# WestlyPark/StyleRenderer

Measured on AMD Instinct MI355X. Metric: generator fwd+bwd images/sec at 256^2, higher is better.
Workload: dtype f32

## Files before the change

stylerenderer_amd/csrc/conv_wino.hip:

```cpp
#include <type_traits>
#include "mfma_tile.h"
#include "conv_wino.h"
#include <cstdlib>

namespace {

__device__ __attribute__((aligned(16))) const float g_wino_zero[4] = {0.f, 0.f, 0.f, 0.f};

constexpr int TW = 16, TH = 4;
constexpr int NB = 64;
constexpr int EH = 2 * TH + 2;
constexpr int LEAD = 3;
constexpr int EWP = 40;
constexpr int PLANE = EH * EWP;

#ifdef WINO_TIMING
__device__ long long g_wino_stamps[8 * 16384];
#define WINO_STAMP(i) do { if (tid == 0) { g_wino_stamps[(blockIdx.x & 16383) * 8 + (i)] = wall_clock64(); } } while (0)
#else
#define WINO_STAMP(i)
#endif

template <int KC>
struct WG {
    static constexpr int CQ = KC / 4;
    static constexpr int PPS = CQ * 512;
    static constexpr int UV = 8 * PPS;
    static constexpr int U_INSTR = UV / 256;
    static constexpr int D_FLOATS = KC * PLANE;
    static constexpr int D_INSTR = (D_FLOATS / 4 + 63) / 64;
    static constexpr int D_BUF = D_INSTR * 256;
    static constexpr int D_PER_WAVE = (D_INSTR + 3) / 4;
    static constexpr int PAD = 4 * UV + 2 * D_BUF;
    static constexpr int STY = PAD + 3 * 256;
};

template <int KC>
__global__ __launch_bounds__(256) void k_conv_wino(const WinoParams p) {
#if __HIP_DEVICE_COMPILE__
    using G = WG<KC>;
    extern __shared__ __attribute__((aligned(16))) float smem[];
    float* const ubuf = smem;
    float* const vbuf = smem + 2 * G::UV;
    float* const dbuf = smem + 4 * G::UV + 1;
    float* const sty = smem + G::STY;

    int bid = sr_xcd_chunk(blockIdx.x, gridDim.x);
    const int slice = bid % p.ks;
    bid /= p.ks;
    const int n_t = bid % p.tiles_n;
    bid /= p.tiles_n;
    const int tx_i = bid % p.tiles_x;
    bid /= p.tiles_x;
    const int ty_i = bid % p.tiles_y;
    const int b = bid / p.tiles_y;
    const int oy0 = ty_i * (2 * TH), ox0 = tx_i * (2 * TW), n0 = n_t * NB;

    const int tid = threadIdx.x, lane = tid & 63;
    const int wave = __builtin_amdgcn_readfirstlane(tid >> 6);
    const int half = lane >> 5, l31 = lane & 31;
    const int wn = wave & 1, wt = wave >> 1;
    const int nchunks = p.kchunks;
    const int k_lo = slice * p.kchunks;
    const int all_chunks = p.C / KC;
    WINO_STAMP(0);
#ifdef WINO_TIMING
    const long long wino_c0 = clock64();
    if (tid == 0) {
        g_wino_stamps[(blockIdx.x & 16383) * 8 + 6] = __builtin_amdgcn_s_getreg((31 << 11) | 4);
        g_wino_stamps[(blockIdx.x & 16383) * 8 + 7] = __builtin_amdgcn_s_getreg((31 << 11) | 20);
    }
#endif

    int d_off[G::D_PER_WAVE];
#pragma unroll
    for (int i = 0; i < G::D_PER_WAVE; ++i) {
        const int j = wave + 4 * i;
        const int f = (j * 64 + lane) * 4;
        int off = SR_BUF_OOB;
        if (j < G::D_INSTR && f < G::D_FLOATS) {
            const int c = f / PLANE, q = f % PLANE;
            const int r = q / EWP, cola = q % EWP;
            const int gy = oy0 - 1 + r, gx = ox0 - 4 + cola;
            if (gy >= 0 && gy < p.H && gx >= 0 && gx + 3 < p.W) off = ((c * p.H + gy) * p.W + gx) * 4;
        }
        d_off[i] = off;
    }
    const int chunk_in_bytes = KC * p.H * p.W * 4;
    const __amdgpu_buffer_rsrc_t r_in = __builtin_amdgcn_make_buffer_rsrc(
        const_cast<float*>(p.in + ((int64_t)b * p.C + (int64_t)k_lo * KC) * p.H * p.W), 0, nchunks * chunk_in_bytes,
        SR_BUF_RSRC_WORD3);
    const __amdgpu_buffer_rsrc_t r_u = __builtin_amdgcn_make_buffer_rsrc(
        const_cast<float*>(p.u + ((int64_t)n_t * all_chunks + k_lo) * G::UV), 0, nchunks * G::UV * 4, SR_BUF_RSRC_WORD3);
    const int u_voff = lane * 16;

    auto dma_d1 = [&](int k, int buf, int i) {
        const int j = wave + 4 * i;
        float* dst = j < G::D_INSTR ? dbuf + buf * G::D_BUF + j * 256 : smem + G::PAD + (wave - 1) * 256;
        __builtin_amdgcn_raw_ptr_buffer_load_lds(r_in, (lptr_t)dst, 16, d_off[i], k * chunk_in_bytes, 0, 0);
    };
    auto dma_u1 = [&](int k, int buf, int i) {
        const int j = wave + 4 * i;
        __builtin_amdgcn_raw_ptr_buffer_load_lds(r_u, (lptr_t)(ubuf + buf * G::UV + j * 256), 16, u_voff,
                                                 (k * G::UV + j * 256) * 4, 0, 0);
    };
    auto dma_d = [&](int k, int buf) {
#pragma unroll
        for (int i = 0; i < G::D_PER_WAVE; ++i) dma_d1(k, buf, i);
    };
    auto dma_u = [&](int k, int buf) {
#pragma unroll
        for (int i = 0; i < G::U_INSTR / 4; ++i) dma_u1(k, buf, i);
    };

    static_assert(KC == 8, "two channel quads per chunk");
    const int t_cq = wave & 1, t_h = wave >> 1;
    const int t_ca = 4 * t_cq + t_h;
    const int t_rd = t_ca * PLANE + (2 * (lane >> 4)) * EWP + LEAD + 2 * (lane & 15);
    const int t_wr = t_cq * 512 + t_h * 128 + lane * 2;

    typedef float f2 __attribute__((ext_vector_type(2)));
    auto ld2 = [](const float* q) { return *reinterpret_cast<const f2*>(q); };
    auto st2 = [](float* q, f2 v) { *reinterpret_cast<f2*>(q) = v; };
    auto pk_add = [](f2 x, f2 y) { f2 r; asm("v_pk_add_f32 %0, %1, %2" : "=v"(r) : "v"(x), "v"(y)); return r; };
    auto pk_sub = [](f2 x, f2 y) {
        f2 r;
        asm("v_pk_add_f32 %0, %1, %2 neg_lo:[0,1] neg_hi:[0,1]" : "=v"(r) : "v"(x), "v"(y));
        return r;
    };
    auto pk_mul_s = [](f2 x, f2 sv, int ch) {
        f2 r;
        if (ch == 0) asm("v_pk_mul_f32 %0, %1, %2 op_sel:[0,0] op_sel_hi:[1,0]" : "=v"(r) : "v"(x), "v"(sv));
        else asm("v_pk_mul_f32 %0, %1, %2 op_sel:[0,1] op_sel_hi:[1,1]" : "=v"(r) : "v"(x), "v"(sv));
        return r;
    };
    auto pk_fms_s = [](f2 x, f2 sv, f2 y, int ch) {
        f2 r;
        if (ch == 0)
            asm("v_pk_fma_f32 %0, %1, %2, %3 op_sel:[0,0,0] op_sel_hi:[1,0,1] neg_lo:[0,0,1] neg_hi:[0,0,1]"
                : "=v"(r) : "v"(x), "v"(sv), "v"(y));
        else
            asm("v_pk_fma_f32 %0, %1, %2, %3 op_sel:[0,1,0] op_sel_hi:[1,1,1] neg_lo:[0,0,1] neg_hi:[0,0,1]"
                : "=v"(r) : "v"(x), "v"(sv), "v"(y));
        return r;
    };
    auto pk_fnma_s = [](f2 x, f2 sv, f2 y, int ch) {
        f2 r;
        if (ch == 0)
            asm("v_pk_fma_f32 %0, %1, %2, %3 op_sel:[0,0,0] op_sel_hi:[1,0,1] neg_lo:[1,0,0] neg_hi:[1,0,0]"
                : "=v"(r) : "v"(x), "v"(sv), "v"(y));
        else
            asm("v_pk_fma_f32 %0, %1, %2, %3 op_sel:[0,1,0] op_sel_hi:[1,1,1] neg_lo:[1,0,0] neg_hi:[1,0,0]"
                : "=v"(r) : "v"(x), "v"(sv), "v"(y));
        return r;
    };
    auto col01 = [](f2 tp, f2 tq) {
        f2 r;
        asm("v_pk_add_f32 %0, %1, %2 op_sel:[0,0] op_sel_hi:[1,0] neg_lo:[0,1] neg_hi:[0,0]" : "=v"(r) : "v"(tp), "v"(tq));
        return r;
    };
    auto col23 = [](f2 tp, f2 tq) {
        f2 r;
        asm("v_pk_add_f32 %0, %1, %2 op_sel:[0,1] op_sel_hi:[1,1] neg_lo:[0,1] neg_hi:[1,0]" : "=v"(r) : "v"(tq), "v"(tp));
        return r;
    };
    struct XF {
        f2 P[2][4], Q[2][4];
        f2 sp[2][2], sq[2][2];
        f2 tp[2][4], tq[2][4];
        f2 o01[2][4], o23[2][4];
    };
    auto xf_read = [&](XF& x, const float* d0, int r) {
#pragma unroll
        for (int ch = 0; ch < 2; ++ch) {
            x.P[ch][r] = ld2(d0 + ch * 2 * PLANE + r * EWP);
            x.Q[ch][r] = ld2(d0 + ch * 2 * PLANE + r * EWP + 2);
        }
    };
    auto xf_step = [&](XF& x, int step, f2 sv) {
#pragma unroll
        for (int ch = 0; ch < 2; ++ch) {
            if (step == 0) {
                x.sp[ch][0] = pk_mul_s(x.P[ch][1], sv, ch);
                x.sp[ch][1] = pk_mul_s(x.P[ch][2], sv, ch);
                x.sq[ch][0] = pk_mul_s(x.Q[ch][1], sv, ch);
                x.sq[ch][1] = pk_mul_s(x.Q[ch][2], sv, ch);
                x.tp[ch][0] = pk_fms_s(x.P[ch][0], sv, x.sp[ch][1], ch);
                x.tq[ch][0] = pk_fms_s(x.Q[ch][0], sv, x.sq[ch][1], ch);
            } else if (step == 1) {
                x.tp[ch][1] = pk_add(x.sp[ch][0], x.sp[ch][1]);
                x.tq[ch][1] = pk_add(x.sq[ch][0], x.sq[ch][1]);
                x.tp[ch][2] = pk_sub(x.sp[ch][1], x.sp[ch][0]);
                x.tq[ch][2] = pk_sub(x.sq[ch][1], x.sq[ch][0]);
                x.tp[ch][3] = pk_fnma_s(x.P[ch][3], sv, x.sp[ch][0], ch);
                x.tq[ch][3] = pk_fnma_s(x.Q[ch][3], sv, x.sq[ch][0], ch);
            } else {
#pragma unroll
                for (int q = 2 * (step - 2); q < 2 * (step - 2) + 2; ++q) {
                    x.o01[ch][q] = col01(x.tp[ch][q], x.tq[ch][q]);
                    x.o23[ch][q] = col23(x.tp[ch][q], x.tq[ch][q]);
                }
            }
        }
    };
    auto xf_write = [&](const XF& x, float* vout, int q) {
#pragma unroll
        for (int ch = 0; ch < 2; ++ch) {
            st2(vout + (2 * q) * G::PPS + ch * 256, x.o01[ch][q]);
            st2(vout + (2 * q + 1) * G::PPS + ch * 256, x.o23[ch][q]);
        }
    };
    auto transform = [&](int k, int dsel, int vsel) {
        const float* d0 = dbuf + dsel * G::D_BUF + t_rd;
        float* v = vbuf + vsel * G::UV + t_wr;
        f2 sv;
        sv.x = sty[k * KC + t_ca];
        sv.y = sty[k * KC + t_ca + 2];
        XF x;
#pragma unroll
        for (int r = 0; r < 4; ++r) xf_read(x, d0, r);
#pragma unroll
        for (int st = 0; st < 4; ++st) xf_step(x, st, sv);
#pragma unroll
        for (int q = 0; q < 4; ++q) xf_write(x, v, q);
    };

    f32x16 acc[16];
#pragma unroll
    for (int pos = 0; pos < 16; ++pos)
#pragma unroll
        for (int r = 0; r < 16; ++r) acc[pos][r] = 0.0f;

    const int a_off = (half * 64 + wn * 32 + l31) * 2;
    const int b_off = (half * 64 + wt * 32 + l31) * 2;

    dma_d(0, 0);
    dma_u(0, 0);
    if (nchunks > 1) dma_d(1, 1);
    for (int c = tid; c < nchunks * KC; c += 256)
        sty[c] = p.iscale ? p.iscale[(int64_t)b * p.C + k_lo * KC + c] : 1.0f;
    __builtin_amdgcn_s_waitcnt(0x0F70);
    __syncthreads();
    WINO_STAMP(1);
    transform(0, 0, 0);
    WINO_STAMP(2);

    static_assert(KC == 8, "the slot schedule below is written for two channel quads per chunk");
    f2 au[2][2][8], bv[2][2][8];
    auto mfma_step = [&](int cq, int m) {
        const int e = m >> 4, pos = m & 15, pp = pos >> 1;
        if (pos & 1) acc[pos] = __builtin_amdgcn_mfma_f32_32x32x2f32(au[cq][e][pp].y, bv[cq][e][pp].y, acc[pos], 0, 0, 0);
        else acc[pos] = __builtin_amdgcn_mfma_f32_32x32x2f32(au[cq][e][pp].x, bv[cq][e][pp].x, acc[pos], 0, 0, 0);
    };
    auto body = [&](int k, auto first_tag) {
        constexpr bool FIRST = decltype(first_tag)::value;
        __builtin_amdgcn_s_waitcnt(0x0F70);
        __syncthreads();
        const int kd = min(k + 2, nchunks - 1), ku = min(k + 1, nchunks - 1);
        const float* ub = ubuf + (k & 1) * G::UV + a_off;
        const float* vb_ = vbuf + (k & 1) * G::UV + b_off;
        const int kn = (k + 1 < nchunks) ? k + 1 : k;
        const float* d0 = dbuf + ((k + 1) & 1) * G::D_BUF + t_rd;
        float* vout = vbuf + ((k + 1) & 1) * G::UV + t_wr;
        f2 sab;
        sab.x = sty[kn * KC + t_ca];
        sab.y = sty[kn * KC + t_ca + 2];
        XF x;
        auto load_ops = [&](int cq, int pp) {
#pragma unroll
            for (int e = 0; e < 2; ++e) {
                au[cq][e][pp] = ld2(ub + pp * G::PPS + cq * 512 + e * 256);
                bv[cq][e][pp] = ld2(vb_ + pp * G::PPS + cq * 512 + e * 256);
            }
        };
#ifndef WINO_RD
#define WINO_RD "0123"
#define WINO_ST "4567"
#define WINO_WR "CDEF"
#define WINO_L0 "4567"
#define WINO_L1 "89AB"
#define WINO_DD "45"
#define WINO_DU "89AB"
#endif
        constexpr char RD[] = WINO_RD, ST[] = WINO_ST, WR[] = WINO_WR, L0[] = WINO_L0, L1[] = WINO_L1, DD[] = WINO_DD,
                       DU[] = WINO_DU;
        static_assert(sizeof(RD) == 5 && sizeof(ST) == 5 && sizeof(WR) == 5 && sizeof(L0) == 5 && sizeof(L1) == 5 &&
                      sizeof(DD) == 3 && sizeof(DU) == 5, "schedule strings");
        static_assert(G::D_PER_WAVE == 4 && G::U_INSTR / 4 == 8, "4 halo + 8 weight DMA instructions per wave");
#pragma unroll
        for (int s = 0; s < 16; ++s) {
            const int cq = (s < 8) ? 1 : 0, j = s & 7;
            const char d = s < 10 ? '0' + s : 'A' + (s - 10);
            if (!(FIRST && s < 8)) {
#pragma unroll
                for (int u = 0; u < 4; ++u) mfma_step(cq, 4 * j + u);
            }
#pragma unroll
            for (int i = 0; i < 4; ++i) {
                if (L0[i] == d) { load_ops(0, 2 * i); load_ops(0, 2 * i + 1); }
                if (L1[i] == d) { load_ops(1, 2 * i); load_ops(1, 2 * i + 1); }
            }
#ifndef WINO_NO_DMA
#pragma unroll
            for (int i = 0; i < 4; ++i) {
                if (i < 2 && DD[i] == d) { dma_d1(kd, k & 1, 2 * i); dma_d1(kd, k & 1, 2 * i + 1); }
                if (DU[i] == d) { dma_u1(ku, (k + 1) & 1, 2 * i); dma_u1(ku, (k + 1) & 1, 2 * i + 1); }
            }
#endif
#ifndef WINO_NO_XFORM
#pragma unroll
            for (int i = 0; i < 4; ++i) if (RD[i] == d) xf_read(x, d0, i);
#pragma unroll
            for (int i = 0; i < 4; ++i) if (ST[i] == d) xf_step(x, i, sab);
#pragma unroll
            for (int i = 0; i < 4; ++i) if (WR[i] == d) xf_write(x, vout, i);
#endif
            __builtin_amdgcn_sched_barrier(0);
        }
    };
    body(0, std::true_type{});
    for (int k = 1; k < nchunks; ++k) body(k, std::false_type{});
#pragma unroll
    for (int m = 0; m < 32; ++m) mfma_step(1, m);

    __builtin_amdgcn_s_waitcnt(0x0F70);
    WINO_STAMP(3);

    const int tile = wt * 32 + l31;
    const int oy = oy0 + 2 * (tile >> 4), ox = ox0 + 2 * (tile & 15);
    const int64_t plane = (int64_t)p.H * p.W;
    float nzv[2][2] = {{0.0f, 0.0f}, {0.0f, 0.0f}};
    if (p.nba && p.nz) {
#pragma clang fp contract(off)
        const float nw = p.nz_w[0];
        const float* nzp = p.nz + b * p.nz_bstride + (int64_t)oy * p.W + ox;
#pragma unroll
        for (int a = 0; a < 2; ++a) {
            nzv[a][0] = nw * nzp[a * p.W];
            nzv[a][1] = nw * nzp[a * p.W + 1];
        }
    }
#pragma unroll
    for (int r = 0; r < 16; ++r) {
        const int n = sr_mfma32_row(r, half, n0 + wn * 32);
        float s[2][4];
#pragma unroll
        for (int j = 0; j < 4; ++j) {
            const float m0 = acc[j][r], m1 = acc[4 + j][r], m2 = acc[8 + j][r], m3 = acc[12 + j][r];
            s[0][j] = (m0 + m1) + m2;
            s[1][j] = (m1 - m2) - m3;
        }
        if (p.ks > 1) {
            float* o = p.partial + (((int64_t)slice * p.B + b) * p.N + n) * plane + (int64_t)oy * p.W + ox;
            *reinterpret_cast<float2*>(o) = make_float2((s[0][0] + s[0][1]) + s[0][2], (s[0][1] - s[0][2]) - s[0][3]);
            *reinterpret_cast<float2*>(o + p.W) = make_float2((s[1][0] + s[1][1]) + s[1][2], (s[1][1] - s[1][2]) - s[1][3]);
            continue;
        }
        const float os = p.oscale ? p.oscale[(int64_t)b * p.N + n] : 1.0f;
        const float ob = p.obias ? p.obias[n] : 0.0f;
        float* o = p.out + ((int64_t)b * p.N + n) * plane + (int64_t)oy * p.W + ox;
        const float ab = (p.nba && p.abias) ? p.abias[n] : 0.0f;
        float y[2][2];
#pragma unroll
        for (int a = 0; a < 2; ++a) {
            const float y0 = (s[a][0] + s[a][1]) + s[a][2];
            const float y1 = (s[a][1] - s[a][2]) - s[a][3];
            float v0 = y0 * os + ob, v1 = y1 * os + ob;
            if (p.nba) {
#pragma clang fp contract(off)
                v0 = v0 + nzv[a][0];
                v1 = v1 + nzv[a][1];
                v0 = v0 + ab;
                v1 = v1 + ab;
                v0 = ((v0 > 0.0f) ? v0 : v0 * p.alpha) * p.gain;
                v1 = ((v1 > 0.0f) ? v1 : v1 * p.alpha) * p.gain;
            }
            y[a][0] = v0;
            y[a][1] = v1;
        }
        *reinterpret_cast<float2*>(o) = make_float2(y[0][0], y[0][1]);
        *reinterpret_cast<float2*>(o + p.W) = make_float2(y[1][0], y[1][1]);
    }
    WINO_STAMP(4);
#ifdef WINO_TIMING
    if (tid == 0) g_wino_stamps[(blockIdx.x & 16383) * 8 + 5] = clock64() - wino_c0;
#endif
#endif
}

__global__ __launch_bounds__(256) void k_wino_reduce(const WinoParams p) {
    const int64_t plane = (int64_t)p.H * p.W, total4 = (int64_t)p.B * p.N * plane / 4;
    const int64_t slab4 = total4;
    for (int64_t i = (int64_t)blockIdx.x * 256 + threadIdx.x; i < total4; i += (int64_t)gridDim.x * 256) {
        const float4* src = reinterpret_cast<const float4*>(p.partial) + i;
        float4 a = src[0];
        for (int s = 1; s < p.ks; ++s) {
            const float4 q = src[s * slab4];
            a.x += q.x; a.y += q.y; a.z += q.z; a.w += q.w;
        }
        const int64_t row = (i * 4) / plane;
        const int n = (int)(row % p.N), b = (int)(row / p.N);
        const int64_t pix = i * 4 - row * plane;
        const float os = p.oscale ? p.oscale[row] : 1.0f;
        const float ob = p.obias ? p.obias[n] : 0.0f;
        float v[4] = {a.x * os + ob, a.y * os + ob, a.z * os + ob, a.w * os + ob};
        if (p.nba) {
#pragma clang fp contract(off)
            const float ab = p.abias ? p.abias[n] : 0.0f;
            float nz[4] = {0.0f, 0.0f, 0.0f, 0.0f};
            if (p.nz) {
                const float nw = p.nz_w[0];
                const float4 q = *reinterpret_cast<const float4*>(p.nz + b * p.nz_bstride + pix);
                nz[0] = nw * q.x; nz[1] = nw * q.y; nz[2] = nw * q.z; nz[3] = nw * q.w;
            }
#pragma unroll
            for (int j = 0; j < 4; ++j) {
                float t = v[j] + nz[j];
                t = t + ab;
                v[j] = ((t > 0.0f) ? t : t * p.alpha) * p.gain;
            }
        }
        reinterpret_cast<float4*>(p.out)[i] = make_float4(v[0], v[1], v[2], v[3]);
    }
}

template <int KC>
__global__ __launch_bounds__(64) void k_wino_weights(float* __restrict__ u, const float* __restrict__ wt, int C,
                                                     int N, int ldw) {
    using G = WG<KC>;
    const int n = blockIdx.x * 64 + threadIdx.x, c = blockIdx.y;
    float g[3][3];
#pragma unroll
    for (int t = 0; t < 9; ++t) g[t / 3][t % 3] = wt[((int64_t)t * C + c) * ldw + n];
    float h[4][3];
#pragma unroll
    for (int j = 0; j < 3; ++j) {
        h[0][j] = g[0][j];
        h[1][j] = 0.5f * ((g[0][j] + g[2][j]) + g[1][j]);
        h[2][j] = 0.5f * ((g[0][j] + g[2][j]) - g[1][j]);
        h[3][j] = g[2][j];
    }
    const int cl = c % KC, cq = cl / 4, e = (cl % 4) / 2, hh = cl % 2;
    float* dst = u + ((int64_t)blockIdx.x * (C / KC) + c / KC) * G::UV + cq * 512 + e * 256 + hh * 128 + threadIdx.x * 2;
#pragma unroll
    for (int i = 0; i < 4; ++i) {
        *reinterpret_cast<float2*>(dst + (2 * i) * G::PPS) = make_float2(h[i][0], 0.5f * ((h[i][0] + h[i][2]) + h[i][1]));
        *reinterpret_cast<float2*>(dst + (2 * i + 1) * G::PPS) = make_float2(0.5f * ((h[i][0] + h[i][2]) - h[i][1]), h[i][2]);
    }
}

template <int KC>
int launch(const WinoParams& p, float* u, const float* wt, int ldw, hipStream_t st, bool u_ready) {
    using G = WG<KC>;
    const int lds = (G::STY + p.kchunks * KC) * 4;
    constexpr auto kern = k_conv_wino<KC>;
    if (!sr_allow_dynamic_lds<kern>(160 * 1024)) return SR_EINVAL;
    if (!u_ready) hipLaunchKernelGGL(k_wino_weights<KC>, dim3(p.N / 64, p.C), dim3(64), 0, st, u, wt, p.C, p.N, ldw);
    const int64_t blocks = (int64_t)p.tiles_n * p.tiles_x * p.tiles_y * p.B * p.ks;
    hipLaunchKernelGGL(kern, dim3((unsigned)blocks), dim3(256), lds, st, p);
    if (p.ks > 1) {
        const int64_t total4 = (int64_t)p.B * p.N * p.H * p.W / 4;
        int64_t grid = (total4 + 255) / 256;
        if (grid > 8192) grid = 8192;
        hipLaunchKernelGGL(k_wino_reduce, dim3((unsigned)grid), dim3(256), 0, st, p);
    }
    return sr_launch_status();
}

}

#ifdef WINO_TIMING
extern "C" int sr_debug_wino_stamps(long long* host, int n) {
    return (int)hipMemcpyFromSymbol(host, HIP_SYMBOL(g_wino_stamps), (size_t)n * sizeof(long long));
}
#endif

bool sr_wino_eligible(int64_t B, int64_t C, int64_t N, int64_t H, int64_t W, const void* in, const void* out) {
    if (B <= 0 || C % 8 != 0 || N % 64 != 0 || H % 8 != 0 || W % 32 != 0) return false;
    if (C > 512 || B * ((W / 32) * (H / 8)) * (N / 64) > 0x7FFFFFFFLL) return false;
    if (C * H * W >= (1LL << 29) - 4 || 16 * C * 64 >= (1LL << 29)) return false;
    return ((reinterpret_cast<uintptr_t>(in) | reinterpret_cast<uintptr_t>(out)) & 15) == 0;
}

int64_t sr_wino_scratch_floats(int64_t C, int64_t N) { return 16 * C * N; }

int sr_wino_split(int64_t B, int64_t C, int64_t N, int64_t H, int64_t W) {
    if (sr_env_off("SR_WINO_SPLIT")) return 1;
    const int64_t blocks = B * (W / (2 * TW)) * (H / (2 * TH)) * (N / NB), nchunks = C / 8;
    int ks = 1;
    while (blocks * ks < 192 && ks < 8 && nchunks % (2 * ks) == 0 && nchunks / (2 * ks) >= 8) ks *= 2;
    return ks;
}
int64_t sr_wino_partial_floats(int64_t B, int64_t C, int64_t N, int64_t H, int64_t W) {
    const int ks = sr_wino_split(B, C, N, H, W);
    return ks > 1 ? (int64_t)ks * B * N * H * W : 0;
}

int sr_wino_conv3x3(float* out, const float* in, const float* wt, int64_t ldw, const float* iscale,
                    const float* oscale, const float* obias, int64_t B, int64_t C, int64_t N, int64_t H, int64_t W,
                    float* u_scratch, hipStream_t st, const WinoNba* nba, bool u_ready) {
    WinoParams p;
    p.in = in; p.u = u_scratch; p.iscale = iscale; p.oscale = oscale; p.obias = obias; p.out = out;
    p.nba = nba ? 1 : 0;
    p.nz = nba ? nba->nz : nullptr; p.nz_w = nba ? nba->nz_w : nullptr; p.abias = nba ? nba->abias : nullptr;
    p.nz_bstride = nba ? nba->nz_bstride : 0; p.alpha = nba ? nba->alpha : 0.0f; p.gain = nba ? nba->gain : 1.0f;
    p.B = (int)B; p.C = (int)C; p.N = (int)N; p.H = (int)H; p.W = (int)W;
    p.tiles_x = (int)(W / (2 * TW)); p.tiles_y = (int)(H / (2 * TH)); p.tiles_n = (int)(N / NB);
    p.ks = sr_wino_split(B, C, N, H, W);
    p.kchunks = (int)(C / 8) / p.ks;
    p.partial = u_scratch + sr_wino_scratch_floats(C, N);
    return launch<8>(p, u_scratch, wt, (int)ldw, st, u_ready);
}
```

stylerenderer_amd/op/conv.py:

```python
import os
import threading

import torch

from .. import _lib
from ._dispatch import hold_for_capture, mark_inputs, native, require_f32, wanted
from . import weight_prep as _wp
from . import wgrad_style as _ws
from .fused_elem import noise_stride, param_grads, rowdot, rowdot_div


PROFILE = None


def _timed(like, kind, geom, flops, launch):
    if PROFILE is None:
        return launch()
    stream = torch.cuda.current_stream(like.device)
    e0, e1 = torch.cuda.Event(enable_timing=True), torch.cuda.Event(enable_timing=True)
    e0.record(stream)
    launch()
    e1.record(stream)
    PROFILE.append((kind, geom, flops, e0, e1))


def conv_out_size(ih, iw, ksize, stride, pad, transposed):
    if transposed:
        return (ih - 1) * stride + ksize - 2 * pad, (iw - 1) * stride + ksize - 2 * pad
    return (ih + 2 * pad - ksize) // stride + 1, (iw + 2 * pad - ksize) // stride + 1


def conv2d_mfma(x, wt, iscale=None, oscale=None, obias=None, ksize=3, stride=1, pad=1,
                transposed=False):
    require_f32(x, "conv2d_mfma")
    require_f32(wt, "conv2d_mfma weight")
    x = x.contiguous()
    b, c, ih, iw = x.shape
    taps, cw, n = wt.shape
    wt, ldw = _wt_pitch(wt)
    if taps != ksize * ksize or cw != c:
        raise RuntimeError("conv2d_mfma: weight must be [k*k, C, N]; got %s for C=%d k=%d"
                           % (tuple(wt.shape), c, ksize))
    oh, ow = conv_out_size(ih, iw, ksize, stride, pad, transposed)
    for t, shape, name in ((iscale, (b, c), "iscale"), (oscale, (b, n), "oscale"), (obias, (n,), "obias")):
        if t is not None:
            require_f32(t, "conv2d_mfma " + name)
            if tuple(t.shape) != shape or not t.is_contiguous():
                raise RuntimeError("conv2d_mfma: %s must be contiguous %s" % (name, shape))
    out = torch.empty((b, n, oh, ow), dtype=x.dtype, device=x.device)
    gh, gw = (ih, iw) if transposed else (oh, ow)
    flops = 2.0 * b * gh * gw * c * n * ksize * ksize
    nscr = _lib.lib().sr_conv2d_scratch_floats(b, c, n, ih, iw, oh, ow, ksize, stride, pad, int(bool(transposed)))
    scratch, flags, entry = _conv_scratch(wt, nscr, (b, c, n, ih, iw, ksize, stride, pad, bool(transposed)), x)
    _timed(x, "conv", (ksize, stride, int(bool(transposed)), b, c, n, gh, gw), flops,
           lambda: native(x).sr_conv2d_mfma_ex(out, x, wt, iscale, oscale, obias, b, c, n, ldw, ih, iw, oh, ow, ksize,
                                               stride, pad, int(bool(transposed)), flags, scratch))
    _scratch_written(entry, b, c, n, ih, iw, x, out)
    return out


class _Scratch:
    __slots__ = ("buf", "ready")

    def __init__(self, buf):
        self.buf, self.ready = buf, False


def _conv_scratch(wt, nscr, key, like):
    if nscr <= 0:
        return None, 0, None
    if not (getattr(wt, "_sr_frozen", False) and key[5:] == (3, 1, 1, False)) or os.environ.get("SR_U_CACHE", "1") == "0":
        return torch.empty(nscr, dtype=like.dtype, device=like.device), 0, None
    cache = wt.__dict__.setdefault("_sr_scratch", {})
    k = key + (os.environ.get("SR_WINOGRAD", "1"), os.environ.get("SR_WINO_SPLIT", "1"), wt._version, wt.data_ptr())
    hit = cache.get(k)
    if hit is None or hit.buf.numel() < nscr:
        if len(cache) >= 6:
            cache.clear()
        hit = cache[k] = _Scratch(torch.empty(nscr, dtype=like.dtype, device=like.device))
    hold_for_capture(hit.buf)
    return hit.buf, (1 if hit.ready else 0), hit


def _scratch_written(entry, b, c, n, h, w, x, out):
    if entry is None or entry.ready:
        return
    if x.is_cuda and torch.cuda.is_current_stream_capturing():
        return
    if _lib.lib().sr_conv2d_uses_winograd(b, c, n, h, w, _lib.ptr(x), _lib.ptr(out)):
        entry.ready = True


class _StyleRequest:
    __slots__ = ("wt", "gis")

    def __init__(self, wt):
        self.wt, self.gis = wt, None


_TLS = threading.local()


def conv2d_wgrad_mfma(x, gy, xscale=None, gscale=None, ksize=3, stride=1, pad=1, transposed=False):
    require_f32(x, "conv2d_wgrad_mfma")
    require_f32(gy, "conv2d_wgrad_mfma grad")
    x = x.contiguous()
    gy = gy.contiguous()
    b, c, ih, iw = x.shape
    b2, n, oh, ow = gy.shape
    if b2 != b or (oh, ow) != conv_out_size(ih, iw, ksize, stride, pad, transposed):
        raise RuntimeError("conv2d_wgrad_mfma: shape mismatch x %s gy %s" % (tuple(x.shape), tuple(gy.shape)))
    for t, shape, name in ((xscale, (b, c), "xscale"), (gscale, (b, n), "gscale")):
        if t is not None and (tuple(t.shape) != shape or not t.is_contiguous() or t.dtype != torch.float32):
            raise RuntimeError("conv2d_wgrad_mfma: %s must be contiguous float32 %s" % (name, shape))
    if (ksize == 1 and stride == 1 and pad == 0 and not transposed and c <= 4 and xscale is None and gscale is None
            and (ih * iw) % 4 == 0 and b * n <= 65535 and n <= 4096 and os.environ.get("SR_WGRAD_SMALL", "1") != "0"):
        from .smallconv import _dw

        return _dw(x, gy).sum(0).view(1, c, n)
    gh, gw = (ih, iw) if transposed else (oh, ow)
    flops = 2.0 * b * gh * gw * c * n * ksize * ksize
    req = getattr(_TLS, "style", None)
    if req is not None and req.gis is None:
        wtp, ldw = _wt_pitch(req.wt)
        dwt, req.gis = _ws.wgrad_style(
            x, gy, xscale, gscale, wtp, ldw, ksize, stride, pad, transposed,
            lambda launch: _timed(x, "wgrad", (ksize, stride, int(bool(transposed)), b, c, n, gh, gw), flops, launch))
        return dwt
    nfl = _lib.lib().sr_conv2d_wgrad_scratch_floats(b, c, n, ih, iw, oh, ow, ksize, stride, pad, int(bool(transposed)))
    if nfl < 0:
        raise RuntimeError("conv2d_wgrad_mfma: unsupported geometry")
    scratch = torch.empty(nfl, dtype=torch.float32, device=x.device)
    dwt = torch.empty((ksize * ksize, c, n), dtype=torch.float32, device=x.device)
    _timed(x, "wgrad", (ksize, stride, int(bool(transposed)), b, c, n, gh, gw), flops,
           lambda: native(x).sr_conv2d_wgrad_mfma(dwt, x, gy, xscale, gscale, b, c, n, ih, iw, oh, ow, ksize, stride, pad,
                                                  int(bool(transposed)), scratch))
    return dwt


_ADJOINT = {"c3": "c3", "c3s2": "t3s2", "t3s2": "c3s2", "c1": "c1"}
_GEOM = {
    "c3": (3, 1, 1, False), "c3s2": (3, 2, 0, False), "t3s2": (3, 2, 0, True), "c1": (1, 1, 0, False),
    "c1s2": (1, 2, 0, False),
}


def adjoint_weight(wt, geom, frozen=False, banked=None):
    if banked is not None and banked[0] == (geom == "c3") and not torch.is_grad_enabled():
        return banked[1]
    if frozen and not wt.requires_grad and not torch.is_grad_enabled():
        return _wp.adjoint_cached(wt, geom == "c3")
    return _wp.adjoint(wt, geom == "c3")


def _bc(s):
    return s[:, :, None, None]


def _input_grads(x, g, wt, iscale, oscale, geom, need_x, need_is, frozen=False, banked=None, fused=True):
    if not (need_x or need_is):
        return None, None
    if geom == "c1s2":
        inner = ConvFn.apply(g, adjoint_weight(wt, "c1", frozen, banked), oscale, None, None, "c1")
        dxu = torch.zeros_like(x)
        dxu[:, :, ::2, ::2] = inner
    else:
        dxu = ConvFn.apply(g, adjoint_weight(wt, geom, frozen, banked), oscale, None, None, _ADJOINT[geom])
    if fused and need_is and need_x:
        gis, gx = rowdot(x, dxu, iscale)
        return gx, gis
    gis = rowdot(x, dxu) if need_is else None
    gx = (dxu * _bc(iscale) if iscale is not None else dxu) if need_x else None
    return gx, gis


STYLE_PATH_COUNTS = {"wgrad": 0, "rowdot": 0}


def _conv_grads(x, g, wt, iscale, oscale, geom, need_x, need_w, need_is, frozen=False, banked=None):
    if (need_w and need_is and iscale is not None and geom in ("c3", "t3s2") and not torch.is_grad_enabled()
            and os.environ.get("SR_STYLE_FROM_WGRAD", "1") != "0" and _ws.part_floats(x, g, *_GEOM[geom]) >= 0):
        STYLE_PATH_COUNTS["wgrad"] += 1
        gx = None
        if need_x:
            gx = ConvFn.apply(g, adjoint_weight(wt, geom, frozen, banked), oscale, iscale, None, _ADJOINT[geom])
        req = _TLS.style = _StyleRequest(wt)
        try:
            gw = conv2d_wgrad_mfma(x, g, iscale, oscale, *_GEOM[geom])
        finally:
            _TLS.style = None
        return gx, gw, req.gis
    if need_is:
        STYLE_PATH_COUNTS["rowdot"] += 1
    gx, gis = _input_grads(x, g, wt, iscale, oscale, geom, need_x, need_is, frozen, banked)
    gw = WgradFn.apply(x, g, iscale, oscale, geom) if need_w else None
    return gx, gw, gis


class ConvFn(torch.autograd.Function):
    @staticmethod
    def forward(ctx, x, wt, iscale, oscale, bias, geom):
        mark_inputs(ctx, x, wt, iscale, oscale, bias, geom)
        k, stride, pad, tr = _GEOM[geom]
        out = conv2d_mfma(x, wt, iscale, oscale, bias, k, stride, pad, tr)
        ctx.frozen = bool(getattr(wt, "_sr_frozen", False))
        ctx.adj = getattr(wt, "_sr_adj", None)
        ctx.geom = geom
        ctx.has = (iscale is not None, oscale is not None, bias is not None)
        ctx.save_for_backward(x, wt, iscale, oscale, bias, out if oscale is not None else None)
        return out

    @staticmethod
    def backward(ctx, g):
        x, wt, iscale, oscale, bias, out = ctx.saved_tensors
        need_x, need_w, need_is, need_os, need_b = wanted(ctx)[:5]
        geom = ctx.geom
        g = g.contiguous()
        gos = gb = None
        gx, gw, gis = _conv_grads(x, g, wt, iscale, oscale, geom, need_x, need_w, need_is, ctx.frozen, ctx.adj)
        if need_os:
            y0 = out - bias[None, :, None, None] if bias is not None else out
            gos = rowdot_div(g, y0, oscale)
        if need_b:
            gb = g.sum((0, 2, 3))
        return gx, gw, gis, gos, gb, None


class WgradFn(torch.autograd.Function):
    @staticmethod
    def forward(ctx, x, g, iscale, oscale, geom):
        mark_inputs(ctx, x, g, iscale, oscale, geom)
        k, stride, pad, tr = _GEOM[geom]
        ctx.geom = geom
        ctx.save_for_backward(x, g, iscale, oscale)
        return conv2d_wgrad_mfma(x, g, iscale, oscale, k, stride, pad, tr)

    @staticmethod
    def backward(ctx, gg):
        x, g, iscale, oscale = ctx.saved_tensors
        need_x, need_g, need_is, need_os = wanted(ctx)[:4]
        geom = ctx.geom
        gg = gg.contiguous()
        g_g = gos = None
        gx, gis = _input_grads(x, g, gg, iscale, oscale, geom, need_x, need_is, fused=False)
        if need_g or need_os:
            dgu = ConvFn.apply(x, gg, iscale, None, None, geom)
            if need_os:
                gos = rowdot(g, dgu)
            if need_g:
                g_g = dgu * _bc(oscale) if oscale is not None else dgu
        return gx, g_g, gis, gos, None


def _aliases(*tensors):
    return [t.view_as(t) if t is not None else None for t in tensors]


def _recorded_backward(saved, needs, gy, rebuild):
    with torch.enable_grad():
        ins = _aliases(*saved)
        y = rebuild(*ins)
        sel = [t for t, nd in zip(ins, needs) if nd and t is not None]
        got = iter(torch.autograd.grad(y, sel, gy, create_graph=True, allow_unused=True)) if sel else iter(())
        grads = [next(got) if (nd and t is not None) else None for t, nd in zip(ins, needs)]
    return tuple(grads) + (None,) * (len(needs) - len(ins))


def conv_nba_shape_ok(x, n, noise):
    if x.device.type != "cuda" or x.dtype != torch.float32 or not x.is_contiguous():
        return False
    b, c, h, w = x.shape
    ok = b * n <= 65535 and _lib.lib().sr_conv2d_path(b, c, n, h, w, h, w, 3, 1, 1, 0, _lib.ptr(x), None, None, 0,
                                                      1) == _lib.CONV_PATH_WINO
    if noise is not None:
        ok = ok and noise.dtype == torch.float32 and noise.numel() in (h * w, b * h * w) and noise.data_ptr() % 16 == 0
    return ok


def conv_nba_supported(x, wt, noise):
    return wt.shape[0] == 9 and conv_nba_shape_ok(x, wt.shape[2], noise)


def _wt_pitch(wt):
    taps, cw, n = wt.shape
    if (wt.stride(2) == 1 and wt.stride(1) % 4 == 0 and wt.stride(1) >= n and wt.stride(0) == cw * wt.stride(1)
            and wt.data_ptr() % 16 == 0):
        return wt, wt.stride(1)
    ldw = (n + 3) // 4 * 4
    return (torch.nn.functional.pad(wt, (0, ldw - n)) if ldw != n else wt.contiguous()), ldw


def _nba_forward(x, wt, iscale, oscale, noise, noise_w, abias, slope, gain):
    b, c, h, w = x.shape
    n = wt.shape[2]
    wtp, ldw = _wt_pitch(wt)
    out = torch.empty((b, n, h, w), dtype=x.dtype, device=x.device)
    nscr = _lib.lib().sr_conv2d_scratch_floats(b, c, n, h, w, h, w, 3, 1, 1, 0)
    scratch, flags, entry = _conv_scratch(wt if wtp is wt else wtp, max(nscr, 1), (b, c, n, h, w, 3, 1, 1, False), x)
    flops = 2.0 * b * h * w * c * n * 9
    _timed(x, "conv", (3, 1, 0, b, c, n, h, w), flops,
           lambda: native(x).sr_conv2d_nba_ex(out, x, wtp, iscale, oscale, noise, noise_w, abias, float(slope),
                                              float(gain), b, c, n, ldw, h, w, noise_stride(noise, h * w), flags,
                                              scratch))
    _scratch_written(entry, b, c, n, h, w, x, out)
    return out


def _nba_backward(saved, cfg, frozen, adj, needs, gy):
    from .fused_elem import _NBA

    x, wt, iscale, oscale, noise, noise_w, abias, out = saved
    slope, gain = cfg
    if torch.is_grad_enabled() and oscale is not None:
        return _recorded_backward(
            (x, wt, iscale, oscale, None, noise_w, abias), needs, gy,
            lambda xa, wa, sa, da, _, nwa, aba: _NBA.apply(ConvFn.apply(xa, wa, sa, da, None, "c3"), noise, nwa, aba,
                                                           slope, gain, out.detach()))
    want_p = bool(needs[6] or (noise is not None and needs[5]))
    if oscale is None:
        from .fused_elem import _NBABackward

        g, gb, gnw = _NBABackward.apply(gy, out, noise, slope, gain, want_p)
        rdot = None
    else:
        g, gb, gnw, rdot = _nba_bwd_dot(gy, out, noise, noise_w, abias, slope, gain, want_p)
    return _nba_grads(saved, frozen, adj, needs, want_p, g, gb, gnw, rdot)


def _nba_grads(saved, frozen, adj, needs, want_p, g, gb, gnw, rdot):
    x, wt, iscale, oscale, noise = saved[:5]
    gos = None
    gx, gw, gis = _conv_grads(x, g, wt, iscale, oscale, "c3", needs[0], needs[1], needs[2], frozen, adj)
    if needs[3] and oscale is not None:
        gos = rdot / oscale
    return (gx, gw, gis, gos, None, (gnw if noise is not None and want_p and needs[5] else None),
            (gb if want_p and needs[6] else None), None, None)


class ConvNBAFn(torch.autograd.Function):
    @staticmethod
    def forward(ctx, x, wt, iscale, oscale, noise, noise_w, abias, slope, gain):
        mark_inputs(ctx, x, wt, iscale, oscale, noise, noise_w, abias, slope, gain)
        out = _nba_forward(x, wt, iscale, oscale, noise, noise_w, abias, slope, gain)
        ctx.save_for_backward(x, wt, iscale, oscale, noise, noise_w, abias, out)
        ctx.cfg = (float(slope), float(gain))
        ctx.frozen = bool(getattr(wt, "_sr_frozen", False))
        ctx.adj = getattr(wt, "_sr_adj", None)
        return out

    @staticmethod
    def backward(ctx, gy):
        return _nba_backward(ctx.saved_tensors, ctx.cfg, ctx.frozen, ctx.adj, wanted(ctx), gy)


def _nba_bwd_dot(gy, out, noise, noise_w, abias, slope, gain, want_params=True):
    gy = gy.contiguous()
    b, n, h, w = out.shape
    inner = h * w
    g = torch.empty_like(out)
    gb, gnw = param_grads(out, noise, want_params)
    rdot = torch.empty((b, n), dtype=out.dtype, device=out.device)
    scratch = torch.empty(_lib.lib().sr_noise_bias_act_bwd_dot_scratch_floats(b, n, inner), dtype=out.dtype,
                          device=out.device)
    native(out).sr_noise_bias_act_bwd_dot(g, gb, gnw, rdot, gy, out, noise, noise_w, abias, slope, gain, b, n, inner,
                                          noise_stride(noise, inner), scratch)
    return g, gb, gnw, rdot


def _blur_bwd_fused():
    import os

    return os.environ.get("SR_BLUR_BWD_FUSED", "1") != "0"


def _blur_nba_bwd(gy, out, k_flipped, p0, shape257, noise, noise_w, abias, slope, gain, want_params=True):
    gy = gy.contiguous()
    b, n, oh, ow = out.shape
    g257 = torch.empty(shape257, dtype=out.dtype, device=out.device)
    gb, gnw = param_grads(out, noise, want_params, zero_empty=False)
    rdot = torch.empty((b, n), dtype=out.dtype, device=out.device)
    scratch = torch.empty(_lib.lib().sr_blur_nba_bwd_scratch_floats(b, n, shape257[2], shape257[3]), dtype=out.dtype,
                          device=out.device)
    native(out).sr_blur_nba_bwd(g257, gb, gnw, rdot, gy, out, k_flipped, noise, noise_w, abias, slope, gain, b, n, oh, ow,
                                shape257[2], shape257[3], p0, noise_stride(noise, oh * ow), scratch)
    return g257, gb, gnw, rdot


def upconv_nba_supported(x, wt, noise, oh, ow):
    b = x.shape[0]
    n = wt.shape[2]
    ok = (x.device.type == "cuda" and x.dtype == torch.float32 and wt.shape[0] == 9 and (oh * ow) % 4 == 0
          and b * n <= 65535)
    if noise is not None:
        ok = ok and noise.dtype == torch.float32 and noise.numel() in (oh * ow, b * oh * ow) and noise.data_ptr() % 16 == 0
    return ok


class UpConvNBAFn(torch.autograd.Function):

    @staticmethod
    def forward(ctx, x, wt, iscale, oscale, kernel, pad, noise, noise_w, abias, slope, gain):
        from .fused_elem import _BlurNBA

        mark_inputs(ctx, x, wt, iscale, oscale, kernel, pad, noise, noise_w, abias, slope, gain)
        y257 = conv2d_mfma(x, wt, iscale, oscale, None, 3, 2, 0, True)
        out = _BlurNBA.forward(_NoCtx(), y257, kernel, pad, noise, noise_w, abias, slope, gain)
        ctx.save_for_backward(x, wt, iscale, oscale, kernel, noise, noise_w, abias, out)
        ctx.cfg = (tuple(pad), float(slope), float(gain), tuple(y257.shape))
        ctx.frozen = bool(getattr(wt, "_sr_frozen", False))
        ctx.adj = getattr(wt, "_sr_adj", None)
        return out

    @staticmethod
    def backward(ctx, gy):
        from .fused_elem import _BlurNBA
        from .upfirdn2d import flipped, upfirdn2d_op

        x, wt, iscale, oscale, kernel, noise, noise_w, abias, out = ctx.saved_tensors
        pad, slope, gain, shape257 = ctx.cfg
        needs = wanted(ctx)
        if torch.is_grad_enabled():
            return _recorded_backward(
                (x, wt, iscale, oscale, None, None, None, noise_w, abias), needs, gy,
                lambda xa, wa, sa, da, _k, _p, _n, nwa, aba: _BlurNBA.apply(
                    ConvFn.apply(xa, wa, sa, da, None, "t3s2"), kernel, pad, noise, nwa, aba, slope, gain, out.detach()))
        want_p = bool(needs[8] or (noise is not None and needs[7]))
        p0 = pad[0]
        oh, ow = out.shape[2], out.shape[3]
        if (_blur_bwd_fused() and pad[0] == pad[1] and shape257[2] == oh + 3 - 2 * p0 and shape257[3] == ow + 3 - 2 * p0
                and tuple(kernel.shape) == (4, 4)):
            g257, gb, gnw, rdot = _blur_nba_bwd(gy, out, flipped(kernel), p0, shape257, noise, noise_w, abias, slope,
                                                gain, want_p)
        else:
            g, gb, gnw, rdot = _nba_bwd_dot(gy, out, noise, noise_w, abias, slope, gain, want_p)
            g257 = upfirdn2d_op(g.reshape(-1, oh, ow, 1), flipped(kernel), 1, 1, 1, 1, 3 - p0,
                                shape257[3] - ow + p0, 3 - p0, shape257[2] - oh + p0).view(shape257)
        gos = None
        gx, gw, gis = _conv_grads(x, g257, wt, iscale, oscale, "t3s2", needs[0], needs[1], needs[2], ctx.frozen, ctx.adj)
        if needs[3] and oscale is not None:
            gos = rdot / oscale
        return (gx, gw, gis, gos, None, None, None, (gnw if noise is not None and want_p and needs[7] else None),
                (gb if want_p and needs[8] else None), None, None)


class _NoCtx:

    def save_for_backward(self, *a):
        pass


def upconv_nba(x, wt, iscale, oscale, kernel, pad, noise, noise_w, abias, slope=0.2, gain=2 ** 0.5):
    return UpConvNBAFn.apply(x, wt, iscale, oscale, kernel, tuple(pad), noise, noise_w, abias, slope, gain)


def conv2d_nba(x, wt, iscale, oscale, noise, noise_w, abias, slope=0.2, gain=2 ** 0.5):
    return ConvNBAFn.apply(x, wt, iscale, oscale, noise, noise_w, abias, slope, gain)


class Conv1x1AddFn(torch.autograd.Function):

    @staticmethod
    def forward(ctx, x, wt, oscale, addend):
        mark_inputs(ctx, x, wt, oscale, addend)
        b, c, h, w = x.shape
        n = wt.shape[2]
        out = torch.empty((b, n, h, w), dtype=x.dtype, device=x.device)
        native(x).sr_conv1x1_add(out, x, wt, oscale, addend, b, c, n, wt.stride(1), h * w)
        ctx.frozen = bool(getattr(wt, "_sr_frozen", False))
        ctx.adj = getattr(wt, "_sr_adj", None)
        ctx.save_for_backward(x, wt, oscale)
        return out

    @staticmethod
    def backward(ctx, g):
        x, wt, oscale = ctx.saved_tensors
        need_x, need_w, _, need_a = wanted(ctx)[:4]
        g = g.contiguous()
        gx = gw = None
        if need_x:
            gx = ConvFn.apply(g, adjoint_weight(wt, "c1", ctx.frozen, ctx.adj), oscale, None, None, "c1")
        if need_w:
            gw = WgradFn.apply(x, g, None, oscale, "c1")
        return gx, gw, None, (g if need_a else None)


def conv1x1_add(x, wt, oscale, addend):
    ok = (x.device.type == "cuda" and x.dtype == torch.float32 and addend.dtype == torch.float32 and x.is_contiguous()
          and addend.is_contiguous() and wt.dim() == 3 and wt.shape[0] == 1 and wt.stride(2) == 1
          and wt.stride(1) % 4 == 0 and (oscale is None or (oscale.is_contiguous() and not oscale.requires_grad))
          and tuple(addend.shape) == (x.shape[0], wt.shape[2], x.shape[2], x.shape[3]))
    if ok:
        b, c, h, w = x.shape
        ok = bool(_lib.lib().sr_conv1x1_add_supported(b, c, wt.shape[2], wt.stride(1), h * w, _lib.ptr(x), _lib.ptr(wt),
                                                      _lib.ptr(addend), _lib.ptr(addend)))
    if not ok:
        return ConvFn.apply(x, wt, None, oscale, None, "c1") + addend
    return Conv1x1AddFn.apply(x, wt, oscale, addend)


def conv2d(x, wt, iscale=None, oscale=None, bias=None, geom="c3"):
    return ConvFn.apply(x, wt, iscale, oscale, bias, geom)
```

Measured before the change: 631.4.

## Add 8x8 Winograd tile variant for 16-wide layers and hoist epilogue loads

Templates the Winograd conv kernel on tile shape and adds an 8x8 tile configuration so that 16-pixel-wide feature maps, previously ineligible because they required width divisible by 32, can use the Winograd path when the layer is large enough. Separately, the epilogue now prefetches per-channel scale, bias and noise values before the final MFMA step and processes output rows in packed pairs using packed f32 adds. The added kernel variant raises code size, and its halo layout costs more LDS per channel. The FLOP threshold keeps small 16x16 layers on the direct path.

```diff
diff --git a/stylerenderer_amd/csrc/conv_wino.hip b/stylerenderer_amd/csrc/conv_wino.hip
--- a/stylerenderer_amd/csrc/conv_wino.hip
+++ b/stylerenderer_amd/csrc/conv_wino.hip
@@ -7,12 +7,8 @@
 
 __device__ __attribute__((aligned(16))) const float g_wino_zero[4] = {0.f, 0.f, 0.f, 0.f};
 
-constexpr int TW = 16, TH = 4;
 constexpr int NB = 64;
-constexpr int EH = 2 * TH + 2;
 constexpr int LEAD = 3;
-constexpr int EWP = 40;
-constexpr int PLANE = EH * EWP;
 
 #ifdef WINO_TIMING
 __device__ long long g_wino_stamps[8 * 16384];
@@ -21,8 +17,13 @@
 #define WINO_STAMP(i)
 #endif
 
-template <int KC>
+template <int KC, int TW_, int TH_>
 struct WG {
+    static constexpr int TW = TW_, TH = TH_;
+    static_assert(TW * TH == 64, "64 tiles per workgroup");
+    static constexpr int EH = 2 * TH + 2;
+    static constexpr int EWP = (LEAD + 2 * TW + 2 + 3) / 4 * 4;
+    static constexpr int PLANE = EH * EWP;
     static constexpr int CQ = KC / 4;
     static constexpr int PPS = CQ * 512;
     static constexpr int UV = 8 * PPS;
@@ -32,13 +33,21 @@
     static constexpr int D_BUF = D_INSTR * 256;
     static constexpr int D_PER_WAVE = (D_INSTR + 3) / 4;
     static constexpr int PAD = 4 * UV + 2 * D_BUF;
-    static constexpr int STY = PAD + 3 * 256;
+    static constexpr int STY = PAD + (4 * D_PER_WAVE - D_INSTR) * 256;
 };
-
-template <int KC>
+using WG16x4 = WG<8, 16, 4>;
+using WG8x8 = WG<8, 8, 8>;
+static_assert(WG16x4::D_INSTR == 13 && WG16x4::STY == 4 * 8192 + 2 * 3328 + 3 * 256, "the 16 x 4 patch as it was");
+static_assert(WG8x8::D_INSTR == 14 && WG8x8::D_BUF * 4 == 14 * 1024, "18 rows x 24 floats per channel: 14 KB of halo");
+constexpr int WINO_MAX_C = 512, WINO_LDS_LIMIT = 160 * 1024;
+static_assert((WG8x8::STY + WINO_MAX_C) * 4 <= WINO_LDS_LIMIT && (WG16x4::STY + WINO_MAX_C) * 4 <= WINO_LDS_LIMIT,
+              "buffers + the style row of 512 channels fit one CU");
+
+template <int KC, int TW, int TH>
 __global__ __launch_bounds__(256) void k_conv_wino(const WinoParams p) {
 #if __HIP_DEVICE_COMPILE__
-    using G = WG<KC>;
+    using G = WG<KC, TW, TH>;
+    constexpr int EWP = G::EWP, PLANE = G::PLANE;
     extern __shared__ __attribute__((aligned(16))) float smem[];
     float* const ubuf = smem;
     float* const vbuf = smem + 2 * G::UV;
@@ -96,7 +105,7 @@
 
     auto dma_d1 = [&](int k, int buf, int i) {
         const int j = wave + 4 * i;
-        float* dst = j < G::D_INSTR ? dbuf + buf * G::D_BUF + j * 256 : smem + G::PAD + (wave - 1) * 256;
+        float* dst = j < G::D_INSTR ? dbuf + buf * G::D_BUF + j * 256 : smem + G::PAD + (j - G::D_INSTR) * 256;
         __builtin_amdgcn_raw_ptr_buffer_load_lds(r_in, (lptr_t)dst, 16, d_off[i], k * chunk_in_bytes, 0, 0);
     };
     auto dma_u1 = [&](int k, int buf, int i) {
@@ -116,7 +125,7 @@
     static_assert(KC == 8, "two channel quads per chunk");
     const int t_cq = wave & 1, t_h = wave >> 1;
     const int t_ca = 4 * t_cq + t_h;
-    const int t_rd = t_ca * PLANE + (2 * (lane >> 4)) * EWP + LEAD + 2 * (lane & 15);
+    const int t_rd = t_ca * PLANE + (2 * (lane / TW)) * EWP + LEAD + 2 * (lane % TW);
     const int t_wr = t_cq * 512 + t_h * 128 + lane * 2;
 
     typedef float f2 __attribute__((ext_vector_type(2)));
@@ -320,66 +329,106 @@
     };
     body(0, std::true_type{});
     for (int k = 1; k < nchunks; ++k) body(k, std::false_type{});
+    __builtin_amdgcn_s_waitcnt(0x0F70);
+    const int tile = wt * 32 + l31;
+    const int oy = oy0 + 2 * (tile / TW), ox = ox0 + 2 * (tile % TW);
+    const int plane = p.H * p.W;
+    const int nrow0 = n0 + wn * 32 + 4 * half;
+    float os[16], ob[16], ab[16], nw = 0.0f, nzr[2][2] = {{0.0f, 0.0f}, {0.0f, 0.0f}};
+#pragma unroll
+    for (int r = 0; r < 16; ++r) { os[r] = 1.0f; ob[r] = 0.0f; ab[r] = 0.0f; }
+    if (p.ks == 1) {
+        if (p.nba && p.nz) {
+            nw = p.nz_w[0];
+            const float* nzp = p.nz + b * p.nz_bstride + (int64_t)oy * p.W + ox;
+#pragma unroll
+            for (int a = 0; a < 2; ++a) {
+                nzr[a][0] = nzp[a * p.W];
+                nzr[a][1] = nzp[a * p.W + 1];
+            }
+        }
+        if (p.oscale) {
+            const float* q = p.oscale + (int64_t)b * p.N + nrow0;
+#pragma unroll
+            for (int r = 0; r < 16; ++r) os[r] = q[sr_mfma32_row(r, 0)];
+        }
+        if (p.obias) {
+#pragma unroll
+            for (int r = 0; r < 16; ++r) ob[r] = p.obias[nrow0 + sr_mfma32_row(r, 0)];
+        }
+        if (p.nba && p.abias) {
+#pragma unroll
+            for (int r = 0; r < 16; ++r) ab[r] = p.abias[nrow0 + sr_mfma32_row(r, 0)];
+        }
+    }
+    __builtin_amdgcn_sched_barrier(0);
 #pragma unroll
     for (int m = 0; m < 32; ++m) mfma_step(1, m);
-
-    __builtin_amdgcn_s_waitcnt(0x0F70);
+    __builtin_amdgcn_sched_barrier(0);
+
     WINO_STAMP(3);
 
-    const int tile = wt * 32 + l31;
-    const int oy = oy0 + 2 * (tile >> 4), ox = ox0 + 2 * (tile & 15);
-    const int64_t plane = (int64_t)p.H * p.W;
     float nzv[2][2] = {{0.0f, 0.0f}, {0.0f, 0.0f}};
     if (p.nba && p.nz) {
 #pragma clang fp contract(off)
-        const float nw = p.nz_w[0];
-        const float* nzp = p.nz + b * p.nz_bstride + (int64_t)oy * p.W + ox;
 #pragma unroll
         for (int a = 0; a < 2; ++a) {
-            nzv[a][0] = nw * nzp[a * p.W];
-            nzv[a][1] = nw * nzp[a * p.W + 1];
-        }
-    }
-#pragma unroll
-    for (int r = 0; r < 16; ++r) {
-        const int n = sr_mfma32_row(r, half, n0 + wn * 32);
-        float s[2][4];
+            nzv[a][0] = nw * nzr[a][0];
+            nzv[a][1] = nw * nzr[a][1];
+        }
+    }
+    float* const obase = p.ks > 1 ? p.partial + (((int64_t)slice * p.B + b) * p.N + n0 + wn * 32) * plane
+                                  : p.out + ((int64_t)b * p.N + n0 + wn * 32) * plane;
+    const unsigned lane_off = (unsigned)(4 * half * plane + oy * p.W + ox);
+#pragma unroll
+    for (int r2 = 0; r2 < 16; r2 += 2) {
+        f2 s[2][4];
 #pragma unroll
         for (int j = 0; j < 4; ++j) {
-            const float m0 = acc[j][r], m1 = acc[4 + j][r], m2 = acc[8 + j][r], m3 = acc[12 + j][r];
-            s[0][j] = (m0 + m1) + m2;
-            s[1][j] = (m1 - m2) - m3;
-        }
-        if (p.ks > 1) {
-            float* o = p.partial + (((int64_t)slice * p.B + b) * p.N + n) * plane + (int64_t)oy * p.W + ox;
-            *reinterpret_cast<float2*>(o) = make_float2((s[0][0] + s[0][1]) + s[0][2], (s[0][1] - s[0][2]) - s[0][3]);
-            *reinterpret_cast<float2*>(o + p.W) = make_float2((s[1][0] + s[1][1]) + s[1][2], (s[1][1] - s[1][2]) - s[1][3]);
-            continue;
-        }
-        const float os = p.oscale ? p.oscale[(int64_t)b * p.N + n] : 1.0f;
-        const float ob = p.obias ? p.obias[n] : 0.0f;
-        float* o = p.out + ((int64_t)b * p.N + n) * plane + (int64_t)oy * p.W + ox;
-        const float ab = (p.nba && p.abias) ? p.abias[n] : 0.0f;
-        float y[2][2];
+            f2 m0, m1, m2, m3;
+            m0.x = acc[j][r2]; m0.y = acc[j][r2 + 1];
+            m1.x = acc[4 + j][r2]; m1.y = acc[4 + j][r2 + 1];
+            m2.x = acc[8 + j][r2]; m2.y = acc[8 + j][r2 + 1];
+            m3.x = acc[12 + j][r2]; m3.y = acc[12 + j][r2 + 1];
+            s[0][j] = pk_add(pk_add(m0, m1), m2);
+            s[1][j] = pk_sub(pk_sub(m1, m2), m3);
+        }
+        f2 yy[2][2];
 #pragma unroll
         for (int a = 0; a < 2; ++a) {
-            const float y0 = (s[a][0] + s[a][1]) + s[a][2];
-            const float y1 = (s[a][1] - s[a][2]) - s[a][3];
-            float v0 = y0 * os + ob, v1 = y1 * os + ob;
-            if (p.nba) {
+            yy[a][0] = pk_add(pk_add(s[a][0], s[a][1]), s[a][2]);
+            yy[a][1] = pk_sub(pk_sub(s[a][1], s[a][2]), s[a][3]);
+        }
+#pragma unroll
+        for (int rr = 0; rr < 2; ++rr) {
+            const int r = r2 + rr;
+            float* o = obase + (size_t)sr_mfma32_row(r, 0) * (size_t)plane + lane_off;
+            if (p.ks > 1) {
+                *reinterpret_cast<float2*>(o) = make_float2(yy[0][0][rr], yy[0][1][rr]);
+                *reinterpret_cast<float2*>(o + p.W) = make_float2(yy[1][0][rr], yy[1][1][rr]);
+                continue;
+            }
+            float y[2][2];
+#pragma unroll
+            for (int a = 0; a < 2; ++a) {
+                const float y0 = yy[a][0][rr];
+                const float y1 = yy[a][1][rr];
+                float v0 = y0 * os[r] + ob[r], v1 = y1 * os[r] + ob[r];
+                if (p.nba) {
 #pragma clang fp contract(off)
-                v0 = v0 + nzv[a][0];
-                v1 = v1 + nzv[a][1];
-                v0 = v0 + ab;
-                v1 = v1 + ab;
-                v0 = ((v0 > 0.0f) ? v0 : v0 * p.alpha) * p.gain;
-                v1 = ((v1 > 0.0f) ? v1 : v1 * p.alpha) * p.gain;
-            }
-            y[a][0] = v0;
-            y[a][1] = v1;
-        }
-        *reinterpret_cast<float2*>(o) = make_float2(y[0][0], y[0][1]);
-        *reinterpret_cast<float2*>(o + p.W) = make_float2(y[1][0], y[1][1]);
+                    v0 = v0 + nzv[a][0];
+                    v1 = v1 + nzv[a][1];
+                    v0 = v0 + ab[r];
+                    v1 = v1 + ab[r];
+                    v0 = ((v0 > 0.0f) ? v0 : v0 * p.alpha) * p.gain;
+                    v1 = ((v1 > 0.0f) ? v1 : v1 * p.alpha) * p.gain;
+                }
+                y[a][0] = v0;
+                y[a][1] = v1;
+            }
+            *reinterpret_cast<float2*>(o) = make_float2(y[0][0], y[0][1]);
+            *reinterpret_cast<float2*>(o + p.W) = make_float2(y[1][0], y[1][1]);
+        }
     }
     WINO_STAMP(4);
 #ifdef WINO_TIMING
@@ -427,7 +476,7 @@
 template <int KC>
 __global__ __launch_bounds__(64) void k_wino_weights(float* __restrict__ u, const float* __restrict__ wt, int C,
                                                      int N, int ldw) {
-    using G = WG<KC>;
+    using G = WG<KC, 16, 4>;
     const int n = blockIdx.x * 64 + threadIdx.x, c = blockIdx.y;
     float g[3][3];
 #pragma unroll
@@ -449,12 +498,13 @@
     }
 }
 
-template <int KC>
+template <int KC, int TW, int TH>
 int launch(const WinoParams& p, float* u, const float* wt, int ldw, hipStream_t st, bool u_ready) {
-    using G = WG<KC>;
+    using G = WG<KC, TW, TH>;
     const int lds = (G::STY + p.kchunks * KC) * 4;
-    constexpr auto kern = k_conv_wino<KC>;
-    if (!sr_allow_dynamic_lds<kern>(160 * 1024)) return SR_EINVAL;
+    constexpr auto kern = k_conv_wino<KC, TW, TH>;
+    if (p.kchunks * KC > WINO_MAX_C || lds > WINO_LDS_LIMIT) return SR_EINVAL;
+    if (!sr_allow_dynamic_lds<kern>(WINO_LDS_LIMIT)) return SR_EINVAL;
     if (!u_ready) hipLaunchKernelGGL(k_wino_weights<KC>, dim3(p.N / 64, p.C), dim3(64), 0, st, u, wt, p.C, p.N, ldw);
     const int64_t blocks = (int64_t)p.tiles_n * p.tiles_x * p.tiles_y * p.B * p.ks;
     hipLaunchKernelGGL(kern, dim3((unsigned)blocks), dim3(256), lds, st, p);
@@ -475,9 +525,23 @@
 }
 #endif
 
+constexpr double WINO_W16_MIN_FLOPS = 2.0e10;
+static_assert(WINO_W16_MIN_FLOPS > 18.0 * 16 * 512 * 512 * 16 * 16, "the 16^2 rows of tests/golden/conv_plan_parent.json stay direct");
+
+static bool wino_w16_wanted(int64_t B, int64_t C, int64_t N, int64_t H, int64_t W) {
+    const int sw = sr_env_char("SR_WINO_W16");
+    if (sw == '0') return false;
+    return sw == 'f' || 18.0 * (double)B * (double)C * (double)N * (double)H * (double)W >= WINO_W16_MIN_FLOPS;
+}
+
+static int64_t wino_blocks(int64_t B, int64_t N, int64_t H, int64_t W) {
+    return W == 16 ? B * (H / 16) * (N / NB) : B * (W / 32) * (H / 8) * (N / NB);
+}
+
 bool sr_wino_eligible(int64_t B, int64_t C, int64_t N, int64_t H, int64_t W, const void* in, const void* out) {
-    if (B <= 0 || C % 8 != 0 || N % 64 != 0 || H % 8 != 0 || W % 32 != 0) return false;
-    if (C > 512 || B * ((W / 32) * (H / 8)) * (N / 64) > 0x7FFFFFFFLL) return false;
+    if (B <= 0 || C % 8 != 0 || N % 64 != 0) return false;
+    if (W == 16 ? (H % 16 != 0 || !wino_w16_wanted(B, C, N, H, W)) : (H % 8 != 0 || W % 32 != 0)) return false;
+    if (C > WINO_MAX_C || wino_blocks(B, N, H, W) > 0x7FFFFFFFLL) return false;
     if (C * H * W >= (1LL << 29) - 4 || 16 * C * 64 >= (1LL << 29)) return false;
     return ((reinterpret_cast<uintptr_t>(in) | reinterpret_cast<uintptr_t>(out)) & 15) == 0;
 }
@@ -486,7 +550,7 @@
 
 int sr_wino_split(int64_t B, int64_t C, int64_t N, int64_t H, int64_t W) {
     if (sr_env_off("SR_WINO_SPLIT")) return 1;
-    const int64_t blocks = B * (W / (2 * TW)) * (H / (2 * TH)) * (N / NB), nchunks = C / 8;
+    const int64_t blocks = wino_blocks(B, N, H, W), nchunks = C / 8;
     int ks = 1;
     while (blocks * ks < 192 && ks < 8 && nchunks % (2 * ks) == 0 && nchunks / (2 * ks) >= 8) ks *= 2;
     return ks;
@@ -495,7 +559,6 @@
     const int ks = sr_wino_split(B, C, N, H, W);
     return ks > 1 ? (int64_t)ks * B * N * H * W : 0;
 }
-
 int sr_wino_conv3x3(float* out, const float* in, const float* wt, int64_t ldw, const float* iscale,
                     const float* oscale, const float* obias, int64_t B, int64_t C, int64_t N, int64_t H, int64_t W,
                     float* u_scratch, hipStream_t st, const WinoNba* nba, bool u_ready) {
@@ -505,9 +568,11 @@
     p.nz = nba ? nba->nz : nullptr; p.nz_w = nba ? nba->nz_w : nullptr; p.abias = nba ? nba->abias : nullptr;
     p.nz_bstride = nba ? nba->nz_bstride : 0; p.alpha = nba ? nba->alpha : 0.0f; p.gain = nba ? nba->gain : 1.0f;
     p.B = (int)B; p.C = (int)C; p.N = (int)N; p.H = (int)H; p.W = (int)W;
-    p.tiles_x = (int)(W / (2 * TW)); p.tiles_y = (int)(H / (2 * TH)); p.tiles_n = (int)(N / NB);
+    const bool w16 = W == 16;
+    p.tiles_x = w16 ? 1 : (int)(W / 32); p.tiles_y = (int)(w16 ? H / 16 : H / 8); p.tiles_n = (int)(N / NB);
     p.ks = sr_wino_split(B, C, N, H, W);
     p.kchunks = (int)(C / 8) / p.ks;
     p.partial = u_scratch + sr_wino_scratch_floats(C, N);
-    return launch<8>(p, u_scratch, wt, (int)ldw, st, u_ready);
-}
+    return w16 ? launch<8, 8, 8>(p, u_scratch, wt, (int)ldw, st, u_ready)
+               : launch<8, 16, 4>(p, u_scratch, wt, (int)ldw, st, u_ready);
+}
diff --git a/stylerenderer_amd/op/conv.py b/stylerenderer_amd/op/conv.py
--- a/stylerenderer_amd/op/conv.py
+++ b/stylerenderer_amd/op/conv.py
@@ -72,7 +72,8 @@
     if not (getattr(wt, "_sr_frozen", False) and key[5:] == (3, 1, 1, False)) or os.environ.get("SR_U_CACHE", "1") == "0":
         return torch.empty(nscr, dtype=like.dtype, device=like.device), 0, None
     cache = wt.__dict__.setdefault("_sr_scratch", {})
-    k = key + (os.environ.get("SR_WINOGRAD", "1"), os.environ.get("SR_WINO_SPLIT", "1"), wt._version, wt.data_ptr())
+    env = os.environ.get
+    k = key + (env("SR_WINOGRAD", "1"), env("SR_WINO_SPLIT", "1"), env("SR_WINO_W16", ""), wt._version, wt.data_ptr())
     hit = cache.get(k)
     if hit is None or hit.buf.numel() < nscr:
         if len(cache) >= 6:
```

After: 635.5, median of 6. No clear change (+0.7%).
